# lis-epfl/apg_trajectory_tracking

Measured on AMD Instinct MI355X. Metric: env-steps/sec (fwd+bwd through dynamics), quad horizon=10 batch=65536, higher is better.
Workload: dtype f32; 1 GPU; quadrotor concurrent rollout fwd+bwd (dynamics + quad_mpc_loss + adjoint), BASELINE configs[1]; batch_per_gpu=65536, global_batch=65536, horizon=10, layout=packed, buffer_sets=20, input_bytes_all_sets=587202560, grad_state0=False, loss_mode=deferred, launch=hip-graph replays of the K steps, <= 1000 steps per graph, replays=3, parallelism=batch-sharded x1, no data-path collective

## Files before the change

apg_trajectory_tracking_amd/_capi.py:

```python
import ctypes
import os

import torch

_HERE = os.path.dirname(os.path.abspath(__file__))
LIB_PATH = os.environ.get("APG_LIB") or os.path.join(_HERE, "csrc", "libapg_hip.so")

LAYOUT_SOA = 0
LAYOUT_AOS = 1
LAYOUT_PACKED = 2
MAX_HORIZON = 48
ROLLOUT_BLOCK = 64

_c_float_p = ctypes.c_void_p


class ApgQuadParams(ctypes.Structure):
    _fields_ = [
        ("mass", ctypes.c_float),
        ("kinv", ctypes.c_float * 3),
        ("inertia", ctypes.c_float * 3),
        ("gravity", ctypes.c_float * 3),
        ("trans_drag", ctypes.c_float * 3),
        ("rot_drag", ctypes.c_float * 3),
# ... 224 lines not shown
        _F, _F, _I, _P, _P, _P, _P, _P, _P, _P],
    "apg_planes_gemm_grouped": [ctypes.POINTER(ApgGemmProblem), _I, _P, _I, _P],
    "apg_to_soa": [_P, _P, _I, _I, _I, _P, _P],
    "apg_to_soa_multi": [ctypes.POINTER(ApgSoaItem), _I, _I, _P],
    "apg_wing_policy_workspace_floats": [],
    "apg_wing_policy_fwd": [_P, _P, ctypes.POINTER(ApgWingPolicy), _I, _I, _P, _P,
                            _P, _P, _P],
    "apg_wing_policy_bwd": [_P, _P, _P, _P, ctypes.POINTER(ApgWingPolicy), _I, _I,
                            _P, _P, _P, _P],
    "apg_linear_wgrad_workspace_floats": [_I, _I],
    "apg_linear_wgrad": [_P, _P, ctypes.c_longlong, _I, _I, _P, _P, _P, _P],
    "apg_wing_learnt_param_count": [],
    "apg_wing_learnt_workspace_floats": [_I],
    "apg_wing_learnt_step_fwd": [
        _P, _P, _F, ctypes.POINTER(ApgWingParams), ctypes.POINTER(ctypes.c_float),
        _I, _P, _P],
    "apg_wing_learnt_step_bwd": [
        _P, _P, _F, ctypes.POINTER(ApgWingParams), ctypes.POINTER(ctypes.c_float),
        _I, _P, _P, _P, _P, _P, _P],
    "apg_wing_mlp_closed_loop": [
        _P, _I, _P, _F, ctypes.POINTER(ApgWingParams),
        ctypes.POINTER(ApgWingPolicy), ctypes.POINTER(ctypes.c_float),
        ctypes.POINTER(ctypes.c_float), _F, _I, _I, _I, _F, _F, _I, _P, _P, _P,
        _P, _P, _P, _P, _P],
    "apg_wing_mlp_closed_loop_env": [
        _P, _I, _P, _F, ctypes.POINTER(ApgWingParams), ctypes.POINTER(ctypes.c_float),
        ctypes.POINTER(ApgLearntResidual),
        ctypes.POINTER(ApgWingPolicy), ctypes.POINTER(ctypes.c_float),
        ctypes.POINTER(ctypes.c_float), _F, _I, _I, _I, _F, _F, _I, _P, _P, _P,
        _P, _P, _P, _P, _P],
    "apg_planes_gemm_workspace_floats": [_I, _I, _I, _I],
    "apg_planes_gemm_default_wgs": [_I, _I, _I, _I],
    "apg_planes_gemm_multi_workspace_floats": [ctypes.POINTER(ApgGemmProblem), _I],
    "apg_planes_gemm_multi": [ctypes.POINTER(ApgGemmProblem), _I, _P, _P],
    "apg_planes_gemm": [_P, _I, _I, _P, _P, _I, _I, _I, _I,
                        ctypes.c_longlong, _P, _I, _P, _I, _P, _P],
    "apg_wing_step_fwd": [_P, _P, _F, ctypes.POINTER(ApgWingParams), _I, _I,
                          _P, _P],
    "apg_wing_step_bwd": [_P, _P, _F, ctypes.POINTER(ApgWingParams), _I, _I,
                          _P, _P, _P, _P],
    "apg_wing_rollout_fwd_bwd": [
        _P, _P, _P, _F, ctypes.POINTER(ApgWingParams),
        ctypes.POINTER(ApgWingLossWeights), _I, _I, _I, _P, _P, _P, _P, _P,
        ctypes.POINTER(ApgDeferredLoss), _P],
    "apg_wing_rollout_fwd": [_P, _P, _F, ctypes.POINTER(ApgWingParams), _I,
                             _I, _I, _P, _P],
    "apg_wing_set_two_per_lane": [_I],
    "apg_cartpole_step_fwd": [_P, _P, _F, ctypes.POINTER(ApgCartpoleParams),
                              _I, _I, _P, _P],
    "apg_cartpole_step_bwd": [_P, _P, _F, ctypes.POINTER(ApgCartpoleParams),
                              _I, _I, _P, _P, _P, _P],
    "apg_cartpole_rollout_fwd_bwd": [
        _P, _P, _F, ctypes.POINTER(ApgCartpoleParams), _I, _I, _I, _P, _P,
        _P, _P, _P, _P],
    "apg_cartpole_rollout_fwd": [_P, _P, _F, ctypes.POINTER(ApgCartpoleParams),
                                 _I, _I, _I, _P, _P],
    "apg_cartpole_policy_workspace_floats": [],
    "apg_cartpole_mlp_closed_loop": [
        _P, _F, ctypes.POINTER(ApgCartpoleParams), ctypes.POINTER(ApgCartpolePolicy),
        _I, _I, _I, _F, _I, _P, _P, _P, _P, _P, _P, _P, _P],
    "apg_cartpole_learnt_param_count": [],
    "apg_cartpole_learnt_workspace_floats": [_I],
    "apg_cartpole_learnt_step_fwd": [_P, _P, _F, ctypes.POINTER(ApgCartpoleLearnt), _I,
                                     _P, _P],
    "apg_cartpole_learnt_step_bwd": [_P, _P, _F, ctypes.POINTER(ApgCartpoleLearnt), _I,
                                     _P, _P, _P, _P, _P, _P],
    "apg_cartpole_learnt_rollout_fwd_bwd": [
        _P, _P, _F, ctypes.POINTER(ApgCartpoleLearnt), _I, _I, _I, _P, _P, _P, _P, _P,
        _P],
    "apg_cartpole_learnt_mlp_closed_loop": [
        _P, _F, ctypes.POINTER(ApgCartpoleLearnt), ctypes.POINTER(ApgCartpolePolicy),
        _I, _I, _I, _F, _I, _P, _P, _P, _P, _P, _P, _P, _P],
    "apg_quad_mpc_solve": [
        _P, _P, _I, _F, ctypes.POINTER(ApgQuadParams),
        ctypes.POINTER(ApgQuadLossWeights), ctypes.POINTER(ApgQuadMpcOptions), _I, _I,
        _P, _P, _P, _P],
    "apg_quad_mpc_closed_loop": [
        _P, _I, _F, ctypes.POINTER(ApgQuadParams), ctypes.POINTER(ApgLearntResidual),
        ctypes.POINTER(ApgQuadParams), ctypes.POINTER(ApgQuadLossWeights),
        ctypes.POINTER(ApgQuadMpcOptions), _I, _I, _I, _F, _F, _I, _P, _P, _P, _P, _P,
        _P, _P, _P],
    "apg_quad_mpc_workspace_floats": [],
    "apg_reduce_loss_partials": [_P, _I, _P, _P],
    "apg_loss_partials_count": [_I],
    "apg_stream_copy": [_P, _P, ctypes.c_longlong, _P],
    "apg_stream_copy_shape": [_P, _P, ctypes.c_longlong, _I, _P],
    "apg_stream_rows_probe": [_P, ctypes.c_longlong, _P, ctypes.c_longlong, _I, _P],
    "apg_version": [],
    "apg_last_error_string": [],
}
_RESTYPES = {"apg_last_error_string": ctypes.c_char_p,
             "apg_planes_gemm_multi_workspace_floats": ctypes.c_longlong,
             "apg_quad_mlp_step_partials_floats": ctypes.c_longlong,
             "apg_quad_mlp_rollout_step_partials_floats": ctypes.c_longlong,
             "apg_linear_wgrad_workspace_floats": ctypes.c_longlong}

_lib = None


def lib():
    global _lib
    if _lib is None:
        if not os.path.exists(LIB_PATH):
            raise RuntimeError(
                f"{LIB_PATH} not found: build it with "
                "`python -m apg_trajectory_tracking_amd.build` "
                "(there is no CPU / PyTorch fallback for the APG kernels)")
        handle = ctypes.CDLL(LIB_PATH)
        for name, argtypes in SIGNATURES.items():
            fn = getattr(handle, name)
            fn.argtypes = argtypes
            fn.restype = _RESTYPES.get(name, ctypes.c_int)
        _lib = handle
    return _lib


def check(code, what):
    if code != 0:
        msg = lib().apg_last_error_string().decode()
        exc = ValueError if code == -1 else RuntimeError
        raise exc(f"{what} failed ({code}): {msg}")


def ptr(t):
    return None if t is None else t.data_ptr()


def stream_of(t):
    return torch.cuda.current_stream(t.device).cuda_stream


def require_device(*tensors):
    dev = None
    for t in tensors:
        if t is None:
            continue
        if not t.is_cuda:
            raise RuntimeError(
                "apg_trajectory_tracking_amd kernels run on an MI355X only: "
                f"got a tensor on {t.device} (no CPU fallback exists)")
        if t.dtype != torch.float32:
            raise TypeError(f"fp32 tensors required, got {t.dtype}")
        if not t.is_contiguous():
            raise ValueError("contiguous tensors required")
        if dev is None:
            dev = t.device
        elif t.device != dev:
            raise RuntimeError("all tensors must live on the same device")
    return dev


def loss_partials_count(B):
    return 1 if B <= 0 else (B + ROLLOUT_BLOCK - 1) // ROLLOUT_BLOCK
```

apg_trajectory_tracking_amd/build.py:

```python
import os
import subprocess
import sys

HERE = os.path.dirname(os.path.abspath(__file__))
REPO = os.path.dirname(HERE)
CSRC = os.path.join(HERE, "csrc")
LIB = os.path.join(CSRC, "libapg_hip.so")
SOURCES = ["common.hip", "quad.hip", "wing.hip", "cartpole.hip", "lstm.hip",
           "mlp_rollout.hip", "mlp_concurrent.hip", "mlp_wing.hip", "wing_learnt.hip",
           "linear_wgrad.hip", "planes_gemm.hip", "mlp_cartpole.hip",
           "cartpole_learnt.hip", "quad_mpc.hip"]
COMMON_FLAGS = ["-fno-slp-vectorize"]
EXTRA_FLAGS = {"quad.hip": ["-mllvm", "-amdgpu-kernarg-preload-count=16"]}
def _headers():
    import glob
    return sorted(glob.glob(os.path.join(CSRC, "*.h"))) + [
        os.path.join(REPO, "include", "apg.h")]


def _stale():
    if not os.path.exists(LIB) or not os.path.exists(
            os.path.join(CSRC, "kernel_resources.json")):
        return True
    t = os.path.getmtime(LIB)
    deps = [os.path.join(CSRC, s) for s in SOURCES] + _headers()
    return any(os.path.exists(d) and os.path.getmtime(d) > t for d in deps)


def _extra_flags():
    flags = os.environ.get("APG_HIPCC_FLAGS", "").split()
    bad = [f for f in flags if f.startswith(("-DAPG_", "-UAPG_"))]
    if bad:
        raise RuntimeError(
            f"APG_HIPCC_FLAGS must not define kernel macros ({' '.join(bad)}): "
            "build variants with tools/build_variant.py")
    return flags


RESOURCES = os.path.join(CSRC, "kernel_resources.json")


def _kernel_resources(remarks):
    import re
    out, cur = {}, None
    keys = {"VGPRs": "vgprs", "AGPRs": "agprs", "TotalSGPRs": "sgprs",
            "ScratchSize [bytes/lane]": "scratch",
            "Occupancy [waves/SIMD]": "occupancy", "VGPRs Spill": "vgpr_spill"}
    for line in remarks.splitlines():
        m = re.search(r"remark: Function Name: (\S+)", line)
        if m:
            cur = out.setdefault(m.group(1), {})
            continue
        m = re.search(r"remark:\s+([A-Za-z][^:]*): (\d+) \[-Rpass-analysis", line)
        if m and cur is not None and m.group(1) in keys:
            cur[keys[m.group(1)]] = int(m.group(2))
    return out


def build(force=False, verbose=False):
    if not force and not _stale():
        return LIB
    extra = _extra_flags()
    hipcc = os.environ.get("HIPCC", "/opt/rocm/bin/hipcc")
    objs = []
    procs = []
    for s in SOURCES:
        src = os.path.join(CSRC, s)
        if not os.path.exists(src):
            continue
        obj = os.path.join(CSRC, s.replace(".hip", ".o"))
        cmd = [hipcc, "--offload-arch=gfx950", "-O3", "-std=c++17", "-fPIC",
               *COMMON_FLAGS, *EXTRA_FLAGS.get(s, []),
               *extra, "-Rpass-analysis=kernel-resource-usage",
               "-I", os.path.join(REPO, "include"), "-I", CSRC, "-c", src,
               "-o", obj]
        if verbose:
            print(" ".join(cmd), file=sys.stderr)
        procs.append((s, subprocess.Popen(
            cmd, stdout=subprocess.PIPE, stderr=subprocess.STDOUT, text=True)))
        objs.append(obj)
    resources = {}
    for s, p in procs:
        out, _ = p.communicate()
        if p.returncode != 0:
            raise RuntimeError(f"hipcc failed on {s}:\n{out}")
        resources.update(_kernel_resources(out))
    import json
    with open(RESOURCES, "w") as f:
        json.dump(resources, f, indent=0, sort_keys=True)
    cmd = [hipcc, "--offload-arch=gfx950", "-shared", "-fPIC", "-o", LIB] + objs
    r = subprocess.run(cmd, stdout=subprocess.PIPE, stderr=subprocess.STDOUT,
                       text=True)
    if r.returncode != 0:
        raise RuntimeError(f"hipcc link failed:\n{r.stdout}")
    return LIB


LIB_CPU = os.path.join(CSRC, "libapg_cpu.so")


def build_cpu(force=False, verbose=False):
    src = os.path.join(CSRC, "cpu_twins.hip")
    deps = [src, os.path.join(REPO, "include", "apg_cpu.h"),
            os.path.join(REPO, "include", "apg_cpu_learnt.h"),
            os.path.join(REPO, "include", "apg_cpu_mpc.h"), __file__] + _headers()
    if (not force and os.path.exists(LIB_CPU)
            and os.path.getmtime(LIB_CPU) >= max(os.path.getmtime(d) for d in deps)):
        return LIB_CPU
    hipcc = os.environ.get("HIPCC", "/opt/rocm/bin/hipcc")
    cmd = [hipcc, "--cuda-host-only", "-no-hip-rt", "-O2", "-std=c++17", "-fPIC",
           "-shared",
           "-I", os.path.join(REPO, "include"), "-I", CSRC, "-o", LIB_CPU, src]
    if verbose:
        print(" ".join(cmd), file=sys.stderr)
    r = subprocess.run(cmd, stdout=subprocess.PIPE, stderr=subprocess.STDOUT, text=True)
    if r.returncode != 0:
        raise RuntimeError(f"hipcc (host) failed on cpu_twins.hip:\n{r.stdout}")
    return LIB_CPU


LIB_PLANES = os.path.join(CSRC, "libapg_planes.so")


def build_planes(force=False, verbose=False):
    srcs = [os.path.join(CSRC, s) for s in ("mlp_planes.hip", "common.hip")]
    deps = srcs + [os.path.join(REPO, "include", "apg_planes.h"), __file__] + _headers()
    if (not force and os.path.exists(LIB_PLANES)
            and os.path.getmtime(LIB_PLANES) >= max(os.path.getmtime(d) for d in deps)):
        return LIB_PLANES
    hipcc = os.environ.get("HIPCC", "/opt/rocm/bin/hipcc")
# ... 16 lines not shown
```

apg_trajectory_tracking_amd/csrc/common.hip:

```cpp
#include <stdarg.h>
#include <stdio.h>

#include "apg_device.h"

namespace apg {

static thread_local char g_err[512] = "";

void set_error(const char *fmt, ...) {
  va_list ap;
  va_start(ap, fmt);
  vsnprintf(g_err, sizeof(g_err), fmt, ap);
  va_end(ap);
}

int device_slot() {
  int d = -1;
  return (hipGetDevice(&d) == hipSuccess && d >= 0 && d < kMaxDevices) ? d : -1;
}

int device_cu_count() {
  static int cus[kMaxDevices] = {};
  const int d = device_slot();
  if (d >= 0 && cus[d] > 0) return cus[d];
  int v = 0;
  if (d < 0 || hipDeviceGetAttribute(&v, hipDeviceAttributeMultiprocessorCount, d) !=
                   hipSuccess || v <= 0) {
    (void)hipGetLastError();
    return 256;
  }
  return cus[d] = v;
}

int check_launch(const char *what) {
  hipError_t e = hipGetLastError();
  if (e == hipSuccess) return APG_OK;
  set_error("%s: HIP error %d (%s)", what, (int)e, hipGetErrorString(e));
  return (e == hipErrorNoDevice || e == hipErrorInvalidDevice) ? APG_ERR_NO_DEVICE
                                                               : APG_ERR_HIP;
}

__global__ __launch_bounds__(256) void reduce_partials_kernel(
    const float *__restrict__ partials, int n, float *__restrict__ out) {
  __shared__ double sm[4];
  double acc = 0.0;
#pragma unroll 4
  for (int i = threadIdx.x; i < n; i += 256) acc += (double)partials[i];
#pragma unroll
  for (int off = 32; off > 0; off >>= 1) acc += __shfl_xor(acc, off, kWave);
  if ((threadIdx.x & 63) == 0) sm[threadIdx.x >> 6] = acc;
  __syncthreads();
  if (threadIdx.x == 0) out[0] = (float)((sm[0] + sm[1]) + (sm[2] + sm[3]));
}

int launch_reduce_partials(const float *partials, int n, float *loss,
                           hipStream_t stream) {
  hipLaunchKernelGGL(reduce_partials_kernel, dim3(1), dim3(256), 0, stream,
                     partials, n, loss);
  return check_launch("reduce_partials");
}

constexpr int kSoaChunk = 128;
struct SoaArgs {
  ApgSoaItem it[APG_SOA_MAX_ITEMS];
  int B;
};

__global__ __launch_bounds__(256) void to_soa_kernel(SoaArgs A) {
  __shared__ float tile[64 * (kSoaChunk + 1)];
  __shared__ long long row_off[64];
  const ApgSoaItem &q = A.it[blockIdx.y];
  const int c0 = blockIdx.z * kSoaChunk;
  if (c0 >= q.R) return;
  const int RC = q.R - c0 < kSoaChunk ? q.R - c0 : kSoaChunk, P = RC + 1;
  const int B = A.B, b0 = blockIdx.x * 64;
  const int nb = B - b0 < 64 ? B - b0 : 64;
  if (threadIdx.x < 64) {
    const int i = threadIdx.x < nb ? threadIdx.x : 0;
    const long long row = q.index ? q.index[b0 + i] : (long long)(b0 + i);
    row_off[threadIdx.x] = row * q.ld;
  }
  __syncthreads();
  const float *__restrict__ src = q.src + c0;
  float *__restrict__ dst = q.dst + (size_t)c0 * B;
  const unsigned magic = RC > 1 ? 0xffffffffu / (unsigned)RC + 1u : 0u;
  const int n = nb * RC;
  for (int e0 = threadIdx.x; e0 < n; e0 += 256 * 8) {
    float v[8];
    int at[8];
#pragma unroll
    for (int k = 0; k < 8; ++k) {
      const int e = e0 + 256 * k;
      const int ee = e < n ? e : 0;
      const int i = RC > 1 ? (int)__umulhi((unsigned)ee, magic) : ee, r = ee - i * RC;
      at[k] = e < n ? i * P + r : -1;
      v[k] = src[row_off[i] + r];
    }
#pragma unroll
    for (int k = 0; k < 8; ++k)
      if (at[k] >= 0) tile[at[k]] = v[k];
  }
  __syncthreads();
  const int x = threadIdx.x & 63, y = threadIdx.x >> 6;
  if (x < nb)
    for (int r = y; r < RC; r += 4) dst[(size_t)r * B + b0 + x] = tile[x * P + r];
}

}

typedef float f32x4_copy __attribute__((ext_vector_type(4)));
static __global__ __launch_bounds__(1024) void copy_flat_kernel(
    const f32x4_copy *__restrict__ src, f32x4_copy *__restrict__ dst, long long n16) {
  const long long i = (long long)blockIdx.x * blockDim.x + threadIdx.x;
  if (i < n16) dst[i] = src[i];
}
template <bool NT>
static __global__ __launch_bounds__(256) void copy_unroll4_kernel(
    const f32x4_copy *__restrict__ src, f32x4_copy *__restrict__ dst, long long n16) {
  const long long stride = (long long)gridDim.x * blockDim.x;
  long long i = (long long)blockIdx.x * blockDim.x + threadIdx.x;
  for (; i + 3 * stride < n16; i += 4 * stride) {
    const f32x4_copy a = src[i], b = src[i + stride], c = src[i + 2 * stride],
                     d = src[i + 3 * stride];
    if (NT) {
      __builtin_nontemporal_store(a, dst + i);
      __builtin_nontemporal_store(b, dst + i + stride);
      __builtin_nontemporal_store(c, dst + i + 2 * stride);
      __builtin_nontemporal_store(d, dst + i + 3 * stride);
    } else {
      dst[i] = a, dst[i + stride] = b, dst[i + 2 * stride] = c, dst[i + 3 * stride] = d;
    }
  }
  for (; i < n16; i += stride) dst[i] = src[i];
}

// ... 126 lines not shown
  hipLaunchKernelGGL(apg::to_soa_kernel, dim3((B + 63) / 64, n, chunks), dim3(256), 0,
                     (hipStream_t)stream, A);
  return apg::check_launch("to_soa");
}

int apg_to_soa(const float *src, const long long *index, int B, int R, int ld,
               float *dst, apg_stream_t stream) {
  const ApgSoaItem item = {src, index, dst, R, ld};
  return apg_to_soa_multi(&item, 1, B, stream);
}

static __global__ __launch_bounds__(256) void stream_copy_kernel(const uint4 *__restrict__ src,
                                                          uint4 *__restrict__ dst,
                                                          long long n16) {
  const long long stride = (long long)gridDim.x * blockDim.x;
  for (long long i = (long long)blockIdx.x * blockDim.x + threadIdx.x; i < n16; i += stride) {
    const uint4 v = src[i];
    __builtin_nontemporal_store(v.x, &dst[i].x);
    __builtin_nontemporal_store(v.y, &dst[i].y);
    __builtin_nontemporal_store(v.z, &dst[i].z);
    __builtin_nontemporal_store(v.w, &dst[i].w);
  }
}

int apg_stream_copy_shape(const void *src, void *dst, long long bytes, int shape,
                          apg_stream_t stream) {
  if (shape == 0) return apg_stream_copy(src, dst, bytes, stream);
  if (!src || !dst || bytes < 0 || (bytes & 15) || ((size_t)src & 15) || ((size_t)dst & 15)) {
    apg::set_error("apg_stream_copy_shape: 16-byte aligned pointers and size expected");
    return APG_ERR_ARG;
  }
  if (shape < 1 || shape > 4) {
    apg::set_error("apg_stream_copy_shape: shape 0..4");
    return APG_ERR_ARG;
  }
  if (bytes == 0) return APG_OK;
  const long long n16 = bytes / 16;
  hipStream_t st = (hipStream_t)stream;
  const f32x4_copy *s_ = (const f32x4_copy *)src;
  f32x4_copy *d_ = (f32x4_copy *)dst;
  if (shape == 1 || shape == 4) {
    const int block = shape == 1 ? 256 : 1024;
    const long long blocks = (n16 + block - 1) / block;
    if (blocks > 0x7fffffffll) { apg::set_error("too large"); return APG_ERR_ARG; }
    hipLaunchKernelGGL(copy_flat_kernel, dim3((unsigned)blocks), dim3(block), 0, st, s_, d_, n16);
  } else {
    long long blocks = (n16 + 255) / 256;
    const long long cap = (long long)apg::device_cu_count() * 8;
    if (blocks > cap) blocks = cap;
    if (shape == 2)
      hipLaunchKernelGGL(copy_unroll4_kernel<false>, dim3((unsigned)blocks), dim3(256), 0, st,
                         s_, d_, n16);
    else
      hipLaunchKernelGGL(copy_unroll4_kernel<true>, dim3((unsigned)blocks), dim3(256), 0, st,
                         s_, d_, n16);
  }
  return apg::check_launch("stream_copy_shape");
}

int apg_stream_copy(const void *src, void *dst, long long bytes, apg_stream_t stream) {
  if (!src || !dst || bytes < 0 || (bytes & 15) || ((size_t)src & 15) || ((size_t)dst & 15)) {
    apg::set_error("apg_stream_copy: 16-byte aligned pointers and size expected");
    return APG_ERR_ARG;
  }
  if (bytes == 0) return APG_OK;
  const long long n16 = bytes / 16;
  long long blocks = (n16 + 255) / 256;
  const long long cap = (long long)apg::device_cu_count() * 8;
  if (blocks > cap) blocks = cap;
  hipLaunchKernelGGL(stream_copy_kernel, dim3((unsigned)blocks), dim3(256), 0,
                     (hipStream_t)stream, (const uint4 *)src, (uint4 *)dst, n16);
  return apg::check_launch("stream_copy");
}

int apg_reduce_loss_partials(const float *partials, int n, float *loss,
                             apg_stream_t stream) {
  if (!partials || !loss || n < 0) {
    apg::set_error("apg_reduce_loss_partials: bad arguments");
    return APG_ERR_ARG;
  }
  return apg::launch_reduce_partials(partials, n, loss, (hipStream_t)stream);
}

int apg_loss_partials_count(int B) {
  return B <= 0 ? 1 : (B + apg::kWave - 1) / apg::kWave;
}

int apg_version(void) { return APG_VERSION_MAJOR * 1000 + APG_VERSION_MINOR; }

const char *apg_last_error_string(void) { return apg::g_err; }

}
```

apg_trajectory_tracking_amd/functional.py:

```python
import ctypes

import torch

from . import _capi
from ._capi import (LAYOUT_AOS, LAYOUT_PACKED, LAYOUT_SOA, check, lib, ptr,
                    require_device, stream_of)

_LAYOUTS = {"aos": LAYOUT_AOS, "soa": LAYOUT_SOA, "packed": LAYOUT_PACKED}


def _layout(layout):
    try:
        return _LAYOUTS[layout]
    except KeyError:
        raise ValueError(
            f"layout must be 'aos', 'soa' or 'packed', got {layout!r}")


def _f32c(t):
    return t.detach().to(torch.float32).contiguous()


QUAD_LOSS_WEIGHTS = dict(pos=10.0, vel=1.0, av=0.1, rates=0.1, thrust=5.0)
WING_LOSS_WEIGHTS = dict(pos=10.0, action=0.1)
# ... 494 lines not shown
        ctx.save_for_backward(s, a, *tensors)
        ctx.meta = (float(dt), bool(residual))
        return out

    @staticmethod
    def backward(ctx, grad_next):
        s, a, *tensors = ctx.saved_tensors
        dt, residual = ctx.meta
        B = s.shape[0]
        g = _f32c(grad_next)
        need = ctx.needs_input_grad
        gs = torch.empty_like(s) if need[0] else None
        ga = torch.empty_like(a) if need[1] else None
        n = lib().apg_cartpole_learnt_param_count()
        gp = torch.empty(n, dtype=torch.float32, device=s.device)
        ws = torch.empty(max(lib().apg_cartpole_learnt_workspace_floats(B), 1),
                         dtype=torch.float32, device=s.device)
        model = _cartpole_learnt_model(tensors, residual)
        check(lib().apg_cartpole_learnt_step_bwd(
            ptr(s), ptr(a), dt, ctypes.byref(model), B, ptr(g), ptr(gs), ptr(ga),
            ptr(gp), ptr(ws), stream_of(s)), "apg_cartpole_learnt_step_bwd")
        parts = list(gp[:6].split(1)) + [gp[6:326].view(64, 5), gp[326:390],
                                         gp[390:646].view(4, 64)]
        grads = [p.view_as(t) if need[4 + i] and (residual or i < 6) else None
                 for i, (p, t) in enumerate(zip(parts, tensors))]
        return (gs, ga, None, None, *grads)


def cartpole_learnt_step(dyn, state, action, dt, residual=True):
    return _CartpoleLearntStep.apply(state, action, dt, residual,
                                     *_cartpole_learnt_tensors(dyn))


def cartpole_learnt_rollout_fwd_bwd(dyn, state0, actions, dt, layout="aos",
                                    want_grad_state0=True, want_states=False,
                                    want_loss=True, out=None):
    lay = _layout(layout)
    if lay == LAYOUT_PACKED:
        raise ValueError("the learnt cart-pole rollout takes 'aos' or 'soa' tensors")
    require_device(state0, actions)
    B, H, A = _seq_shape(actions, lay)
    if A != 1 or _state_batch(state0, lay) != B:
        raise ValueError("inconsistent rollout shapes")
    o = _alloc_outs(out, state0.device, B, H, 4, 1, lay, state0, actions,
                    want_grad_state0, want_states, want_loss)
    model = _cartpole_learnt_model(_cartpole_learnt_tensors(dyn))
    check(lib().apg_cartpole_learnt_rollout_fwd_bwd(
        ptr(state0), ptr(actions), float(dt), ctypes.byref(model), B, H, lay,
        ptr(o["loss_partials"]), ptr(o["loss"]), ptr(o["grad_actions"]),
        ptr(o["grad_state0"]), ptr(o["states"]), stream_of(state0)),
        "apg_cartpole_learnt_rollout_fwd_bwd")
    return o


class _CartpoleLearntRolloutLoss(torch.autograd.Function):
    @staticmethod
    def forward(ctx, state0, action_seq, dt, dyn):
        s, a = _f32c(state0), _f32c(action_seq)
        res = cartpole_learnt_rollout_fwd_bwd(
            dyn, s, a, dt, want_grad_state0=ctx.needs_input_grad[0])
        ctx.save_for_backward(res["grad_actions"], res["grad_state0"])
        return res["loss"].reshape(())

    @staticmethod
    def backward(ctx, g):
        ga, gs = ctx.saved_tensors
        ga = ga * g if ctx.needs_input_grad[1] else None
        gs = gs * g if (gs is not None and ctx.needs_input_grad[0]) else None
        return gs, ga, None, None


def cartpole_learnt_rollout_loss(dyn, state0, action_seq, dt):
    return _CartpoleLearntRolloutLoss.apply(state0, action_seq, dt, dyn)


def reduce_loss_partials(partials, loss=None):
    require_device(partials, loss)
    if loss is None:
        loss = torch.empty(1, dtype=torch.float32, device=partials.device)
    check(lib().apg_reduce_loss_partials(
        ptr(partials), partials.numel(), ptr(loss), stream_of(partials)),
        "apg_reduce_loss_partials")
    return loss


class RolloutPlan:

    def __init__(self, system, state0, actions, ref, dt, params, weights=None,
                 layout="soa", want_grad_state0=False, want_states=False,
                 loss_mode="eager", out=None):
        if loss_mode not in ("eager", "deferred", "none"):
            raise ValueError("loss_mode must be eager, deferred or none")
        self.system = system
        self.layout = layout
        self.loss_mode = loss_mode
        self.inputs = (state0, actions, ref)
        kw = dict(layout=layout, want_grad_state0=want_grad_state0,
                  want_states=want_states, want_loss=True, out=out)
        if system == "quad":
            self.out = quad_rollout_fwd_bwd(state0, actions, ref, dt, params,
                                            weights, **kw)
            weights = weights or quad_loss_weights()
            fn = lib().apg_quad_rollout_fwd_bwd
        elif system == "wing":
            self.out = wing_rollout_fwd_bwd(state0, actions, ref, dt, params,
                                            weights, **kw)
            weights = weights or wing_loss_weights()
            fn = lib().apg_wing_rollout_fwd_bwd
        else:
            raise ValueError("system must be 'quad' or 'wing'")
        lay = _layout(layout)
        B, H, _ = _seq_shape(actions, lay)
        self.B, self.H = B, H
        self._keep = [params, weights]
        o = self.out
        head = [ptr(state0), ptr(actions), ptr(ref)]
        if system == "quad":
            head.append(_seq_shape(ref, lay)[2])
        self._fn = fn
        self._head = head + [
            float(dt), ctypes.byref(params), ctypes.byref(weights), B, H, lay,
            ptr(o["loss_partials"]),
            ptr(o["loss"]) if loss_mode == "eager" else None,
            ptr(o["grad_actions"]), ptr(o["grad_state0"]), ptr(o["states"])]
        self._stream = stream_of(state0)
        self._args = tuple(self._head + [None, self._stream])
        self._args_after = {}

    def _deferred_args(self, prev):
        key = id(prev)
        args = self._args_after.get(key)
        if args is None:
            d = _capi.ApgDeferredLoss(
                ptr(prev.out["loss_partials"]),
                prev.out["loss_partials"].numel(), ptr(prev.out["loss"]))
            self._keep.append(d)
            args = tuple(self._head + [ctypes.byref(d), self._stream])
            self._args_after[key] = args
        return args

    def launch(self, after=None):
        args = self._args if after is None else self._deferred_args(after)
        code = self._fn(*args)
        if code != 0:
            check(code, "fused rollout launch")
        return self.out

    def flush(self):
        reduce_loss_partials(self.out["loss_partials"], self.out["loss"])
        return self.out["loss"]


POLICY_INPUT_LIMIT = 16384.0
CHECK_POLICY_INPUT_RANGE = True


class _RangeGuard:
    def __init__(self, slots=32):
        self.slots, self.seen = slots, []

    def __call__(self, what, **tensors):
        if not CHECK_POLICY_INPUT_RANGE:
            return
        import weakref
        fresh = []
        for name, t in tensors.items():
            if t is None or not torch.is_tensor(t) or t.numel() == 0:
                continue
            if any(r() is t and v == t._version for r, v in self.seen):
                continue
            fresh.append((name, t))
        if not fresh or (fresh[0][1].is_cuda and torch.cuda.is_current_stream_capturing()):
            return
        amax = torch.stack([t.detach().abs().amax().float() for _, t in fresh]).tolist()
        for (name, t), m in zip(fresh, amax):
            if not m < POLICY_INPUT_LIMIT:
                raise ValueError(
                    f"{what}: `{name}` holds a value of magnitude {m:g}; the "
                    f"in-kernel policy takes finite inputs below "
                    f"{POLICY_INPUT_LIMIT:g} (fp16-split operands, include/apg.h "
                    "\"operand range\") - normalise the data or use the "
                    "PyTorch policy path (fused_policy = False)")
            self.seen.append((weakref.ref(t), t._version))
        self.seen = [e for e in self.seen if e[0]() is not None][-self.slots:]


_guard_policy_inputs = _RangeGuard()


_GEMM_WGS = None
_bdesc_cache = {}


class _BDesc:
    __slots__ = ("tensor", "base_plane", "J", "host")

    def __init__(self, tensor, base_plane, J, host):
        self.tensor, self.base_plane, self.J, self.host = tensor, base_plane, J, host

    def span(self, S, sdiv):
        q, r = (S - 1) // sdiv, min(S, sdiv) - 1
        return 1 + max(o + q * a + r * b for o, a, b in zip(*self.host))

    @property
    def shape(self):
        return self.tensor.shape

    def data_ptr(self):
        return self.tensor.data_ptr()


def make_bdesc(dev, offsets, stride1=0, stride2=0, key=None):
    k = (str(dev), key)
    if key is not None and k in _bdesc_cache:
        return _bdesc_cache[k]
    offsets = [int(o) for o in offsets]
    J = len(offsets)
    bc = lambda v: [int(x) for x in v] if hasattr(v, "__len__") else [int(v)] * J
    s1, s2 = bc(stride1), bc(stride2)
    if min(s1) < 0 or min(s2) < 0 or min(offsets) < 0:
        raise ValueError("make_bdesc: plane offsets and strides must be >= 0")
    base = min(offsets)
    host = ([o - base for o in offsets], s1, s2)
    t = torch.tensor(list(host), dtype=torch.int32, device=dev)
    d = _BDesc(t, base, J, host)
    if key is not None:
        _bdesc_cache[k] = d
    return d


def _b_operand(Bp, bdesc, N, S, sdiv):
    planes = bdesc.span(S, sdiv)
# ... 1431 lines not shown
```

include/apg.h:

```cpp
#ifndef APG_H_
#define APG_H_

#ifdef __cplusplus
extern "C" {
#endif

#define APG_VERSION_MAJOR 0
#define APG_VERSION_MINOR 1

typedef void *apg_stream_t;
typedef void *apg_event_t;

enum { APG_LAYOUT_SOA = 0, APG_LAYOUT_AOS = 1, APG_LAYOUT_PACKED = 2 };

enum {
  APG_OK = 0,
  APG_ERR_ARG = -1,
  APG_ERR_HIP = -2,
  APG_ERR_NO_DEVICE = -3
};

#ifndef APG_ROLLOUT_BLOCK
#define APG_ROLLOUT_BLOCK 64
#endif
// ... 419 lines not shown
                         float *states_out, apg_stream_t stream);
int apg_wing_set_two_per_lane(int mode);

typedef struct ApgCartpoleParams {
  float masscart, masspole, length, max_force_mag, friction, gravity;
} ApgCartpoleParams;

int apg_cartpole_step_fwd(const float *state, const float *action, float dt,
                          const ApgCartpoleParams *params, int B, int layout,
                          float *next_state, apg_stream_t stream);
int apg_cartpole_step_bwd(const float *state, const float *action, float dt,
                          const ApgCartpoleParams *params, int B, int layout,
                          const float *grad_next, float *grad_state,
                          float *grad_action, apg_stream_t stream);

int apg_cartpole_rollout_fwd_bwd(const float *state0, const float *actions,
                                 float dt, const ApgCartpoleParams *params,
                                 int B, int H, int layout,
                                 float *loss_partials, float *loss,
                                 float *grad_actions, float *grad_state0,
                                 float *states_out, apg_stream_t stream);

int apg_cartpole_rollout_fwd(const float *state0, const float *actions, float dt,
                             const ApgCartpoleParams *params, int B, int H,
                             int layout, float *states_out, apg_stream_t stream);

typedef struct ApgCartpolePolicy {
  const float *w0;
  const float *b0;
  const float *w1;
  const float *b1;
  const float *w2;
  const float *b2;
  const float *w3;
  const float *b3;
  const float *w_out;
  const float *b_out;
} ApgCartpolePolicy;

enum { APG_CARTPOLE_BALANCE = 0, APG_CARTPOLE_SWINGUP = 1 };

int apg_cartpole_policy_workspace_floats(void);
int apg_cartpole_mlp_closed_loop(const float *state0, float dt,
                                 const ApgCartpoleParams *params,
                                 const ApgCartpolePolicy *policy, int B, int max_steps,
                                 int mode, float thresh_div, int burn_in, int *steps,
                                 int *upright, double *vel_sum, double *vel_sq,
                                 float *states, float *actions, float *workspace,
                                 apg_stream_t stream);

typedef struct ApgCartpoleLearnt {
  const float *max_force_mag, *masspole, *length, *friction, *total_mass,
      *polemass_length, *w1, *b1, *w2;
} ApgCartpoleLearnt;

int apg_cartpole_learnt_param_count(void);
int apg_cartpole_learnt_workspace_floats(int B);
int apg_cartpole_learnt_step_fwd(const float *state, const float *action, float dt,
                                 const ApgCartpoleLearnt *model, int B, float *next_state,
                                 apg_stream_t stream);
int apg_cartpole_learnt_step_bwd(const float *state, const float *action, float dt,
                                 const ApgCartpoleLearnt *model, int B,
                                 const float *grad_next, float *grad_state,
                                 float *grad_action, float *grad_params, float *workspace,
                                 apg_stream_t stream);

int apg_cartpole_learnt_rollout_fwd_bwd(const float *state0, const float *actions, float dt,
                                        const ApgCartpoleLearnt *model, int B, int H,
                                        int layout, float *loss_partials, float *loss,
                                        float *grad_actions, float *grad_state0,
                                        float *states_out, apg_stream_t stream);

int apg_cartpole_learnt_mlp_closed_loop(const float *state0, float dt,
                                        const ApgCartpoleLearnt *model,
                                        const ApgCartpolePolicy *policy, int B,
                                        int max_steps, int mode, float thresh_div,
                                        int burn_in, int *steps, int *upright,
                                        double *vel_sum, double *vel_sq, float *states,
                                        float *actions, float *workspace,
                                        apg_stream_t stream);

int apg_reduce_loss_partials(const float *partials, int n, float *loss,
                             apg_stream_t stream);
int apg_to_soa(const float *src, const long long *index, int B, int R, int ld,
               float *dst, apg_stream_t stream);
#define APG_SOA_MAX_ITEMS 6
typedef struct ApgSoaItem {
  const float *src;
  const long long *index;
  float *dst;
  int R, ld;
} ApgSoaItem;
int apg_to_soa_multi(const ApgSoaItem *items, int n, int B, apg_stream_t stream);
int apg_loss_partials_count(int B);
int apg_stream_copy(const void *src, void *dst, long long bytes, apg_stream_t stream);
int apg_stream_copy_shape(const void *src, void *dst, long long bytes, int shape,
                          apg_stream_t stream);
int apg_stream_rows_probe(const void *in, long long in_bytes, void *out, long long out_bytes,
                          int shape, apg_stream_t stream);

int apg_version(void);
const char *apg_last_error_string(void);

#ifdef __cplusplus
}
#endif
#endif
```

Measured before the change: 77.51 billion env-steps/s.

## Add launch chain planner for deferred-loss rollouts with optional two-stream lanes

Adds a host-side launch chain that tracks the pending loss partials for each stream lane and works out fork, join and cross-lane event edges. Deferred rollout launches can then alternate across two streams and fold the previous step's loss reduction into the next launch. With the default CHAIN_LANES=1 everything stays on the caller stream, and the chain mostly replaces the per-pair ApgDeferredLoss caching with C-side bookkeeping. In exchange, each launch now makes an extra ctypes call for begin_step, and the added event logic is more complex.

Result: no change. 77.38 billion env-steps/s (-0.2%).

```diff
diff --git a/apg_trajectory_tracking_amd/_capi.py b/apg_trajectory_tracking_amd/_capi.py
--- a/apg_trajectory_tracking_amd/_capi.py
+++ b/apg_trajectory_tracking_amd/_capi.py
@@ -330,6 +330,14 @@
         _P, _P, _P],
     "apg_quad_mpc_workspace_floats": [],
     "apg_reduce_loss_partials": [_P, _I, _P, _P],
+    "apg_chain_create": [_I, ctypes.POINTER(ctypes.c_void_p)],
+    "apg_chain_destroy": [_P],
+    "apg_chain_begin_step": [_P, _P, _I, _I, _P, _P, _I, _P,
+                             ctypes.POINTER(ctypes.c_void_p),
+                             ctypes.POINTER(ApgDeferredLoss)],
+    "apg_chain_abort_step": [_P],
+    "apg_chain_flush": [_P, _P],
+    "apg_chain_steps": [_P],
     "apg_loss_partials_count": [_I],
     "apg_stream_copy": [_P, _P, ctypes.c_longlong, _P],
     "apg_stream_copy_shape": [_P, _P, ctypes.c_longlong, _I, _P],
diff --git a/apg_trajectory_tracking_amd/build.py b/apg_trajectory_tracking_amd/build.py
--- a/apg_trajectory_tracking_amd/build.py
+++ b/apg_trajectory_tracking_amd/build.py
@@ -45,7 +45,8 @@
     out, cur = {}, None
     keys = {"VGPRs": "vgprs", "AGPRs": "agprs", "TotalSGPRs": "sgprs",
             "ScratchSize [bytes/lane]": "scratch",
-            "Occupancy [waves/SIMD]": "occupancy", "VGPRs Spill": "vgpr_spill"}
+            "Occupancy [waves/SIMD]": "occupancy", "VGPRs Spill": "vgpr_spill",
+            "LDS Size [bytes/block]": "lds"}
     for line in remarks.splitlines():
         m = re.search(r"remark: Function Name: (\S+)", line)
         if m:
diff --git a/apg_trajectory_tracking_amd/csrc/common.hip b/apg_trajectory_tracking_amd/csrc/common.hip
--- a/apg_trajectory_tracking_amd/csrc/common.hip
+++ b/apg_trajectory_tracking_amd/csrc/common.hip
@@ -2,6 +2,7 @@
 #include <stdio.h>
 
 #include "apg_device.h"
+#include "launch_chain_plan.h"
 
 namespace apg {
 
@@ -40,8 +41,8 @@
                                                                : APG_ERR_HIP;
 }
 
-__global__ __launch_bounds__(256) void reduce_partials_kernel(
-    const float *__restrict__ partials, int n, float *__restrict__ out) {
+__device__ __forceinline__ void reduce_partials_block(const float *__restrict__ partials,
+                                                      int n, float *__restrict__ out) {
   __shared__ double sm[4];
   double acc = 0.0;
 #pragma unroll 4
@@ -51,6 +52,20 @@
   if ((threadIdx.x & 63) == 0) sm[threadIdx.x >> 6] = acc;
   __syncthreads();
   if (threadIdx.x == 0) out[0] = (float)((sm[0] + sm[1]) + (sm[2] + sm[3]));
+}
+
+__global__ __launch_bounds__(256) void reduce_partials_kernel(
+    const float *__restrict__ partials, int n, float *__restrict__ out) {
+  reduce_partials_block(partials, n, out);
+}
+
+struct ReduceJobs {
+  const float *partials[kChainMaxLanes];
+  float *out[kChainMaxLanes];
+  int n[kChainMaxLanes];
+};
+__global__ __launch_bounds__(256) void reduce_partials_multi_kernel(ReduceJobs J) {
+  reduce_partials_block(J.partials[blockIdx.x], J.n[blockIdx.x], J.out[blockIdx.x]);
 }
 
 int launch_reduce_partials(const float *partials, int n, float *loss,
@@ -343,6 +358,168 @@
   return apg::launch_reduce_partials(partials, n, loss, (hipStream_t)stream);
 }
 
+struct ApgLaunchChain {
+  apg::ChainPlan plan;
+  apg::ChainPlan before;
+  int device;
+  hipStream_t caller;
+  hipStream_t helper;
+  hipEvent_t fork, join;
+  hipEvent_t cross[apg::kChainMaxLanes];
+};
+
+static int chain_hip_error(const char *what) {
+  const int rc = apg::check_launch(what);
+  if (rc) return rc;
+  apg::set_error("%s failed", what);
+  return APG_ERR_HIP;
+}
+#define APG_CHAIN_HIP(call, what)                                              \
+  do {                                                                         \
+    if ((call) != hipSuccess) return chain_hip_error(what);                    \
+  } while (0)
+#define APG_CHAIN_TRY(call, what)                                              \
+  do {                                                                         \
+    if ((call) != hipSuccess) {                                                \
+      chain->plan = saved;                                                     \
+      return chain_hip_error(what);                                            \
+    }                                                                          \
+  } while (0)
+
+static hipStream_t chain_lane(const ApgLaunchChain *c, int lane) {
+  return lane == 0 ? c->caller : c->helper;
+}
+
+int apg_chain_create(int device, ApgLaunchChain **chain) {
+  if (!chain) { apg::set_error("apg_chain_create: chain is NULL"); return APG_ERR_ARG; }
+  *chain = nullptr;
+  int cur = -1;
+  APG_CHAIN_HIP(hipGetDevice(&cur), "apg_chain_create: hipGetDevice");
+  if (device < 0) device = cur;
+  if (device != cur) APG_CHAIN_HIP(hipSetDevice(device), "apg_chain_create: hipSetDevice");
+  ApgLaunchChain *c = new ApgLaunchChain();
+  c->device = device;
+  bool ok = hipStreamCreateWithFlags(&c->helper, hipStreamNonBlocking) == hipSuccess;
+  hipEvent_t *ev[] = {&c->fork, &c->join, &c->cross[0], &c->cross[1]};
+  for (hipEvent_t *e : ev)
+    ok = ok && hipEventCreateWithFlags(e, hipEventDisableTiming) == hipSuccess;
+  int rc = ok ? APG_OK : apg::check_launch("apg_chain_create: stream / events");
+  if (device != cur) (void)hipSetDevice(cur);
+  if (!ok) {
+    apg_chain_destroy(c);
+    return rc ? rc : APG_ERR_HIP;
+  }
+  *chain = c;
+  return APG_OK;
+}
+
+int apg_chain_destroy(ApgLaunchChain *chain) {
+  if (!chain) return APG_OK;
+  hipEvent_t ev[] = {chain->fork, chain->join, chain->cross[0], chain->cross[1]};
+  for (hipEvent_t e : ev)
+    if (e) (void)hipEventDestroy(e);
+  if (chain->helper) (void)hipStreamDestroy(chain->helper);
+  (void)hipGetLastError();
+  delete chain;
+  return APG_OK;
+}
+
+int apg_chain_steps(const ApgLaunchChain *chain) {
+  return chain ? (int)(chain->plan.steps() > 0x7fffffffl ? 0x7fffffffl : chain->plan.steps()) : 0;
+}
+
+int apg_chain_flush(ApgLaunchChain *chain, apg_stream_t stream) {
+  if (!chain) { apg::set_error("apg_chain_flush: chain is NULL"); return APG_ERR_ARG; }
+  if (chain->plan.idle()) return APG_OK;
+  if ((hipStream_t)stream != chain->caller) {
+    apg::set_error("apg_chain_flush: not the stream the chain was begun on");
+    return APG_ERR_ARG;
+  }
+  const apg::ChainPlan saved = chain->plan;
+  const apg::ChainFlush f = chain->plan.flush();
+  if (f.join) {
+    APG_CHAIN_TRY(hipEventRecord(chain->join, chain->helper), "apg_chain_flush: record");
+    APG_CHAIN_TRY(hipStreamWaitEvent(chain->caller, chain->join, 0), "apg_chain_flush: wait");
+  }
+  if (f.n_reduce == 1) {
+    const int e = apg::launch_reduce_partials(f.reduce[0].partials, f.reduce[0].count,
+                                              f.reduce[0].loss, chain->caller);
+    if (e) chain->plan = saved;
+    return e;
+  }
+  if (f.n_reduce > 1) {
+    apg::ReduceJobs J;
+    for (int i = 0; i < f.n_reduce; ++i)
+      J.partials[i] = f.reduce[i].partials, J.n[i] = f.reduce[i].count,
+      J.out[i] = f.reduce[i].loss;
+    hipLaunchKernelGGL(apg::reduce_partials_multi_kernel, dim3(f.n_reduce), dim3(256), 0,
+                       chain->caller, J);
+    const int e = apg::check_launch("reduce_partials_multi");
+    if (e) chain->plan = saved;
+    return e;
+  }
+  return APG_OK;
+}
+
+int apg_chain_abort_step(ApgLaunchChain *chain) {
+  if (!chain) { apg::set_error("apg_chain_abort_step: chain is NULL"); return APG_ERR_ARG; }
+  chain->plan = chain->before;
+  return APG_OK;
+}
+
+int apg_chain_begin_step(ApgLaunchChain *chain, apg_stream_t stream, int lanes, int restart,
+                         const void *out_key, const float *loss_partials, int n_partials,
+                         float *loss, apg_stream_t *lane, ApgDeferredLoss *fold) {
+  if (!chain || !lane || !fold || !loss_partials || !loss || n_partials < 0) {
+    apg::set_error("apg_chain_begin_step: chain / lane / fold / loss_partials / loss NULL "
+                   "or n_partials < 0");
+    return APG_ERR_ARG;
+  }
+  if (lanes < 1 || lanes > apg::kChainMaxLanes) {
+    apg::set_error("apg_chain_begin_step: lanes must be 1 or %d", apg::kChainMaxLanes);
+    return APG_ERR_ARG;
+  }
+  if (!chain->plan.idle()) {
+    if (restart) {
+      if (int e = apg_chain_flush(chain, chain->caller)) return e;
+    } else if ((hipStream_t)stream != chain->caller) {
+      apg::set_error("apg_chain_begin_step: not the stream the chain was begun on");
+      return APG_ERR_ARG;
+    }
+  }
+  if (chain->plan.idle()) chain->caller = (hipStream_t)stream;
+  const apg::ChainPlan saved = chain->plan;
+  chain->before = saved;
+  const apg::ChainDecision d =
+      chain->plan.begin_step(lanes, out_key, loss_partials, n_partials, loss);
+  const hipStream_t ls = chain_lane(chain, d.lane);
+  if (d.fork)
+    APG_CHAIN_TRY(hipEventRecord(chain->fork, chain->caller), "apg_chain_begin_step: fork");
+  if (d.lane_start)
+    APG_CHAIN_TRY(hipStreamWaitEvent(ls, chain->fork, 0), "apg_chain_begin_step: fork wait");
+  for (int i = 0; i < d.n_reduce; ++i)
+    if (int e = apg::launch_reduce_partials(d.reduce[i].partials, d.reduce[i].count,
+                                            d.reduce[i].loss,
+                                            chain_lane(chain, d.reduce_lane[i]))) {
+      chain->plan = saved;
+      return e;
+    }
+  if (d.cross_edge) {
+    const int other = 1 - d.lane;
+    APG_CHAIN_TRY(hipEventRecord(chain->cross[other], chain_lane(chain, other)),
+                  "apg_chain_begin_step: cross record");
+    APG_CHAIN_TRY(hipStreamWaitEvent(ls, chain->cross[other], 0),
+                  "apg_chain_begin_step: cross wait");
+  }
+  *lane = (apg_stream_t)ls;
+  fold->prev_partials = d.fold.partials;
+  fold->prev_count = d.fold.count;
+  fold->prev_loss = d.fold.loss;
+  return APG_OK;
+}
+#undef APG_CHAIN_HIP
+#undef APG_CHAIN_TRY
+
 int apg_loss_partials_count(int B) {
   return B <= 0 ? 1 : (B + apg::kWave - 1) / apg::kWave;
 }
diff --git a/apg_trajectory_tracking_amd/csrc/launch_chain_plan.h b/apg_trajectory_tracking_amd/csrc/launch_chain_plan.h
--- /dev/null
+++ b/apg_trajectory_tracking_amd/csrc/launch_chain_plan.h
@@ -0,0 +1,119 @@
+#ifndef APG_LAUNCH_CHAIN_PLAN_H_
+#define APG_LAUNCH_CHAIN_PLAN_H_
+
+namespace apg {
+
+constexpr int kChainMaxLanes = 2;
+constexpr int kChainKeys = 64;
+
+struct ChainPartials {
+  const float *partials;
+  int count;
+  float *loss;
+};
+
+struct ChainDecision {
+  int lane;
+  bool fork;
+  bool lane_start;
+  int n_reduce;
+  int reduce_lane[kChainMaxLanes];
+  ChainPartials reduce[kChainMaxLanes];
+  bool cross_edge;
+  ChainPartials fold;
+};
+
+struct ChainFlush {
+  int n_reduce;
+  ChainPartials reduce[kChainMaxLanes];
+  bool join;
+};
+
+class ChainPlan {
+ public:
+  ChainPlan() { reset(); }
+
+  bool idle() const { return steps_ == 0; }
+  int lanes() const { return lanes_; }
+  long steps() const { return steps_; }
+
+  ChainDecision begin_step(int lanes_wanted, const void *key, const float *partials,
+                           int count, float *loss) {
+    if (steps_ == 0)
+      lanes_ = lanes_wanted < 1 ? 1 : lanes_wanted > kChainMaxLanes ? kChainMaxLanes
+                                                                    : lanes_wanted;
+    ChainDecision d = {};
+    const int lane = (int)(steps_ % lanes_);
+    d.lane = lane;
+    d.fork = steps_ == 0 && lanes_ > 1;
+    d.lane_start = lane != 0 && !lane_used_[lane];
+    bool other_touched = false;
+    for (int l = 0; l < lanes_; ++l) {
+      ChainPartials &p = pending_[l];
+      if (p.partials && (p.partials == partials || p.loss == loss)) {
+        d.reduce_lane[d.n_reduce] = l;
+        d.reduce[d.n_reduce++] = p;
+        p = ChainPartials{nullptr, 0, nullptr};
+        other_touched |= l != lane;
+      }
+    }
+    const int at = find(key);
+    const bool other_ran = lanes_ > 1 && lane_used_[1 - lane];
+    if (at >= 0)
+      d.cross_edge = key_lane_[at] != lane;
+    else
+      d.cross_edge = overflow_ && other_ran;
+    d.cross_edge = (d.cross_edge || other_touched) && other_ran;
+    d.fold = pending_[lane];
+    pending_[lane] = ChainPartials{partials, count, loss};
+    lane_used_[lane] = true;
+    if (at >= 0) {
+      key_lane_[at] = lane;
+    } else if (n_keys_ < kChainKeys) {
+      keys_[n_keys_] = key;
+      key_lane_[n_keys_++] = lane;
+    } else {
+      overflow_ = true;
+    }
+    ++steps_;
+    return d;
+  }
+
+  ChainFlush flush() {
+    ChainFlush f = {};
+    for (int l = 0; l < lanes_; ++l)
+      if (pending_[l].partials) f.reduce[f.n_reduce++] = pending_[l];
+    f.join = lanes_ > 1 && lane_used_[1];
+    reset();
+    return f;
+  }
+
+ private:
+  void reset() {
+    lanes_ = 1;
+    steps_ = 0;
+    n_keys_ = 0;
+    overflow_ = false;
+    for (int l = 0; l < kChainMaxLanes; ++l) {
+      lane_used_[l] = false;
+      pending_[l] = ChainPartials{nullptr, 0, nullptr};
+    }
+  }
+  int find(const void *key) const {
+    for (int i = 0; i < n_keys_; ++i)
+      if (keys_[i] == key) return i;
+    return -1;
+  }
+
+  int lanes_;
+  long steps_;
+  bool lane_used_[kChainMaxLanes];
+  ChainPartials pending_[kChainMaxLanes];
+  const void *keys_[kChainKeys];
+  int key_lane_[kChainKeys];
+  int n_keys_;
+  bool overflow_;
+};
+
+}
+#endif
diff --git a/apg_trajectory_tracking_amd/functional.py b/apg_trajectory_tracking_amd/functional.py
--- a/apg_trajectory_tracking_amd/functional.py
+++ b/apg_trajectory_tracking_amd/functional.py
@@ -600,6 +600,34 @@
         ptr(partials), partials.numel(), ptr(loss), stream_of(partials)),
         "apg_reduce_loss_partials")
     return loss
+
+
+CHAIN_LANES = 1
+
+
+class _LaunchChain:
+
+    def __init__(self, device_index):
+        self.handle = ctypes.c_void_p()
+        check(lib().apg_chain_create(device_index, ctypes.byref(self.handle)),
+              "apg_chain_create")
+        self.lane = ctypes.c_void_p()
+        self.fold = _capi.ApgDeferredLoss()
+        self.lane_ref = ctypes.byref(self.lane)
+        self.fold_ref = ctypes.byref(self.fold)
+        self.lanes = 1
+
+
+_CHAINS = {}
+
+
+def _launch_chain(dev, stream):
+    index = dev.index if dev.index is not None else torch.cuda.current_device()
+    key = (index, stream)
+    chain = _CHAINS.get(key)
+    if chain is None:
+        chain = _CHAINS[key] = _LaunchChain(index)
+    return chain
 
 
 class RolloutPlan:
@@ -643,29 +671,44 @@
             ptr(o["grad_actions"]), ptr(o["grad_state0"]), ptr(o["states"])]
         self._stream = stream_of(state0)
         self._args = tuple(self._head + [None, self._stream])
-        self._args_after = {}
-
-    def _deferred_args(self, prev):
-        key = id(prev)
-        args = self._args_after.get(key)
-        if args is None:
-            d = _capi.ApgDeferredLoss(
-                ptr(prev.out["loss_partials"]),
-                prev.out["loss_partials"].numel(), ptr(prev.out["loss"]))
-            self._keep.append(d)
-            args = tuple(self._head + [ctypes.byref(d), self._stream])
-            self._args_after[key] = args
-        return args
+        self._chain = None
+        if loss_mode == "deferred":
+            self._chain = chain = _launch_chain(state0.device, self._stream)
+            self._begin = lib().apg_chain_begin_step
+            self._begin_args = (
+                ptr(o["grad_actions"]), ptr(o["loss_partials"]),
+                o["loss_partials"].numel(), ptr(o["loss"]), chain.lane_ref, chain.fold_ref)
+            self._head = tuple(self._head)
 
     def launch(self, after=None):
-        args = self._args if after is None else self._deferred_args(after)
-        code = self._fn(*args)
+        chain = self._chain
+        if chain is None:
+            code = self._fn(*self._args)
+            if code != 0:
+                check(code, "fused rollout launch")
+            return self.out
+        if after is None:
+            chain.lanes = 2 if CHAIN_LANES >= 2 else 1
+        elif after is self:
+            raise ValueError("a plan cannot defer its loss onto its own launch")
+        elif after._chain is not chain:
+            raise ValueError("`after` must be a deferred plan made on the same stream")
+        code = self._begin(chain.handle, self._stream, chain.lanes, after is None,
+                           *self._begin_args)
+        if code == 0:
+            code = self._fn(*self._head, chain.fold_ref, chain.lane.value)
+            if code != 0:
+                lib().apg_chain_abort_step(chain.handle)
         if code != 0:
             check(code, "fused rollout launch")
         return self.out
 
     def flush(self):
-        reduce_loss_partials(self.out["loss_partials"], self.out["loss"])
+        chain = self._chain
+        if chain is not None and lib().apg_chain_steps(chain.handle) > 0:
+            check(lib().apg_chain_flush(chain.handle, self._stream), "apg_chain_flush")
+        else:
+            reduce_loss_partials(self.out["loss_partials"], self.out["loss"])
         return self.out["loss"]
 
 
diff --git a/include/apg.h b/include/apg.h
--- a/include/apg.h
+++ b/include/apg.h
@@ -525,6 +525,15 @@
 
 int apg_reduce_loss_partials(const float *partials, int n, float *loss,
                              apg_stream_t stream);
+typedef struct ApgLaunchChain ApgLaunchChain;
+int apg_chain_create(int device, ApgLaunchChain **chain);
+int apg_chain_destroy(ApgLaunchChain *chain);
+int apg_chain_begin_step(ApgLaunchChain *chain, apg_stream_t stream, int lanes, int restart,
+                         const void *out_key, const float *loss_partials, int n_partials,
+                         float *loss, apg_stream_t *lane, ApgDeferredLoss *fold);
+int apg_chain_abort_step(ApgLaunchChain *chain);
+int apg_chain_flush(ApgLaunchChain *chain, apg_stream_t stream);
+int apg_chain_steps(const ApgLaunchChain *chain);
 int apg_to_soa(const float *src, const long long *index, int B, int R, int ld,
                float *dst, apg_stream_t stream);
 #define APG_SOA_MAX_ITEMS 6
```
